# fabriceo/AVDSP

Hardware: AMD Instinct MI355X
Metric: Msamples/s (all ch) biquad+FIR chain (higher is better)
Workload: dtype f64; 1 GPU; north: 4096 ch x (16 biquads + 4096-tap FIR), block 1024 frames, DSP_FORMAT 6; 4096 ch in total, 4096 ch/GPU by dspRuntimeSetShard(rank, 1), no data-path collective; channels=4096, channels_per_gpu=4096, taps=4096, block=1024, format=6, overlap=1, ready_words=-1, ready_mode=2, side_by_side=1, streams_remade=0, cu_split=0, fir_split=0, fir_launch=-1, fir_lean=-1, ring_wait=1

## Files before the change

### avdsp_amd/csrc/avdsp_kernels.hip

```cpp
#include <hip/hip_runtime.h>
#include <hip/hip_ext.h>
#include <atomic>
#include <chrono>
#include <mutex>
#include <thread>

#include <cstdarg>
#include <cstdio>
#include <cstring>
#include <type_traits>
#include <utility>
#include <vector>
#include <algorithm>

#include "avdsp_hip.h"
#include "avdsp_format.h"

namespace {

thread_local char g_err[512];
thread_local bool g_err_ready = false;

int set_err(const char *fmt, ...)
{
// ... 1367 lines not shown

template <int FMT>
__device__ __forceinline__ void fir_append_input(const FirArgs &a, const avdsp_chain &c, int cid)
{
    const int B = a.io.nframes;
    const unsigned *inp = a.io.in + (c.in_io - a.io.in_base);
    for (int q = threadIdx.x; q < B; q += blockDim.x) {
        unsigned raw = inp[(size_t)q * a.io.in_stride];
        if constexpr (FMT == 6) raw = ftz_bits(raw);
        ring_put(a.ring, cid, q, ftz_bits(narrow_stage<FMT>(load_stage<FMT>(raw, c.load_mode, c.gain_bits))));
    }
    __syncthreads();
}

struct ChunkRegs { float h[kHRegs], x[kWRegs]; };

__device__ __forceinline__ int fir_win_slot(int u, int tid)
{
    const int idx = u * kBlock + tid, i = idx & 15, t = idx >> 4;
    return 16 * (16 * (t >> 4) + i) + (t & 15);
}

__device__ __forceinline__ void fir_chunk_fetch(const FirArgs &a, const avdsp_chain &c, int cid, int mlo, ChunkRegs &r)
{
    const int T = c.fir_taps, B = a.io.nframes, tid = threadIdx.x;
    const float *taps = reinterpret_cast<const float *>(a.buf + c.fir_coef_word);
    const float *ringrow = ring_row(a.ring, cid);
    const int rmask = a.ring.R - 1, wlen = fir_win_len(a.gpc), woff = fir_win_off(a.gpc);
#pragma unroll
    for (int u = 0; u < kHRegs; u++) { const int t = mlo + u * kBlock + tid; r.h[u] = (t >= 0 && t < T) ? taps[t] : 0.0f; }
#pragma unroll
    for (int u = 0; u < kWRegs; u++) {
        const int w = fir_win_slot(u, tid), q = w - mlo - woff;
        r.x[u] = (w < wlen && q < B) ? ringrow[(a.ring.wpos + q) & rmask] : 0.0f;
    }
}

__device__ __forceinline__ void fir_chunk_to_lds(const FirArgs &a, const ChunkRegs &r, double *hs, double *xs, int row)
{
    const int tid = threadIdx.x, hlen = fir_hs_len(a.gpc), wlen = fir_win_len(a.gpc);
#pragma unroll
    for (int u = 0; u < kHRegs; u++) { const int i = u * kBlock + tid; if (i < hlen) hs[i] = mulop(r.h[u]); }
#pragma unroll
    for (int u = 0; u < kWRegs; u++) { const int w = fir_win_slot(u, tid); if (w < wlen) xs[win_pos(w, row)] = mulop(r.x[u]); }
}

typedef double v4f64 __attribute__((ext_vector_type(4)));
typedef double v2f64 __attribute__((ext_vector_type(2)));

template <int FMT, int NG>
__global__ __launch_bounds__(kBlock, NG == 1 ? 5 : 4) void fir_mfma(const FirArgs a)
{
    extern __shared__ __attribute__((aligned(16))) double lds[];
    const int slot = xcd_remap(blockIdx.x, a.per_xcd);
    if (slot >= a.ngroup) return;
    const int cid = a.group[slot];
    const avdsp_chain c = a.chains[cid];
    double *hs = lds, *xs = lds + a.hs_cap;
    const int row = a.win_row, gpc = a.gpc;
    const int T = c.fir_taps, B = a.io.nframes;
    if (c.nsec == 0) fir_append_input<FMT>(a, c, cid);

    const int lane = threadIdx.x & 63, wave = threadIdx.x >> 6;
    const int ij = lane & 15, k = lane >> 4;
    const bool busy = wave * kTileFrames < B;
    const double *hp = hs + k + ij;
    const double *xp[4];
    const int f0 = 16 * 16 * wave + fir_win_off(gpc) - k;
#pragma unroll
    for (int s = 0; s < 4; s++) xp[s] = xs + win_pos(f0 - 4 * s, row) + ij;
    v4f64 acc = {0.0, 0.0, 0.0, 0.0};

    double ha[4 * NG], xa[4 * NG], hb[4 * NG], xb[4 * NG];
    auto load_set = [&](double *h, double *x, int g) {
#pragma unroll
        for (int q = 0; q < NG; q++)
#pragma unroll
            for (int s = 0; s < 4; s++) { h[4 * q + s] = hp[16 * (g + q) + 4 * s]; x[4 * q + s] = xp[s][-(g + q)]; }
    };
    auto mfma_set = [&](const double *h, const double *x) {
#pragma unroll
        for (int u = 0; u < 4 * NG; u++) acc = __builtin_amdgcn_mfma_f64_16x16x4f64(h[u], x[u], acc, 0, 0, 0);
    };

    const int total_groups = (T + 15 + 15) >> 4;
    const int phase = (blockIdx.x >> 8) & 3;
    int glen = max(NG, (gpc * (phase + 1) / 4) / NG * NG);
    ChunkRegs regs;
    fir_chunk_fetch(a, c, cid, -15, regs);
    for (int g0 = 0; g0 < total_groups; g0 += glen, glen = gpc) {
        __syncthreads();
        fir_chunk_to_lds(a, regs, hs, xs, row);
        __syncthreads();
        if (g0 + glen < total_groups) fir_chunk_fetch(a, c, cid, -15 + 16 * (g0 + glen), regs);
        if (busy) {
            const int ng = min(glen, total_groups - g0);
            const int nsets = (ng + NG - 1) / NG;
            load_set(ha, xa, 0);
            int st = 0;
            for (; st + 2 <= nsets; st += 2) {
                load_set(hb, xb, NG * (st + 1));
                __builtin_amdgcn_sched_barrier(0);
                mfma_set(ha, xa);
                __builtin_amdgcn_sched_barrier(0);
                load_set(ha, xa, NG * (st + 2));
                __builtin_amdgcn_sched_barrier(0);
                mfma_set(hb, xb);
                __builtin_amdgcn_sched_barrier(0);
            }
            if (st < nsets) mfma_set(ha, xa);
        }
    }
#pragma unroll
    for (int r = 0; r < 4; r++) {
        const int n = 16 * (16 * wave + ij) + k + 4 * r;
        if (n < B) {
            unsigned word = store_stage<FMT>(acc[r], c.sat, a.io.store_mask);
            if constexpr (FMT == 6) word = ftz_bits(word);
            emit_out(a.io, c, n, word);
        }
    }
}


constexpr int kTapsLead = 64;
constexpr int kTapsTail = 384;
__host__ __device__ inline int taps64_pitch(int max_taps) { return (kTapsLead + max_taps + kTapsTail + 1) & ~1; }

template <int R, bool BIG = false> struct TileGeom {
    static_assert(!BIG || R == 1, "long chunks: one row tile");
    static constexpr int NR = 16 * R;
    static constexpr int FW = 256 * R;
    static constexpr int WPC = 4 / R;
    static constexpr int QD = 4 * (R - 1);
    static constexpr int CKMAX = R == 4 ? 96 : R == 2 ? 128 : BIG ? 320 : 160;
    static constexpr int ROW = R == 4 ? 23 : R == 2 ? 33 : BIG ? 97 : 57;
    static constexpr int HNEED = 4 * CKMAX + 16 * (R - 1) + 28;
    static constexpr int HLEN = (HNEED + 127) / 128 * 128;
    static constexpr int WLEN = NR * ROW + (NR * ROW & 1);
    static constexpr int LDS_DOUBLES = 2 * HLEN + WLEN;
    static constexpr int NW = (NR * ROW + 63) / 64;
};
static_assert(TileGeom<4>::ROW >= 16 + (4 * (TileGeom<4>::CKMAX - 1) + 63) / 64 && TileGeom<2>::ROW >= 16 + (4 * (TileGeom<2>::CKMAX - 1) + 31) / 32 &&
              TileGeom<1>::ROW >= 16 + (4 * (TileGeom<1>::CKMAX - 1) + 15) / 16 &&
              TileGeom<1, true>::ROW >= 16 + (4 * (TileGeom<1, true>::CKMAX - 1) + 15) / 16, "window rows hold a chunk");

struct FirTileArgs {
    int *buf; const avdsp_chain *chains; const int *group; int ngroup; Ring ring; int per_xcd;
    const double *taps64; int pitch64;
    BlockIO io;
    unsigned *ready; unsigned seq; unsigned *timeouts;
    int ready_acquire;
    int wpc_shift;
#ifdef AVDSP_FIR_STAMPS
    unsigned long long *stamps;
#endif
};
#ifdef AVDSP_FIR_STAMPS
#define FIR_STAMP(i) do { if (lane == 0 && (i) <= 30) a.stamps[(size_t)(blockIdx.x * 4 + stamp_row) * 32 + (i)] = __builtin_amdgcn_s_memtime(); } while (0)
#define FIR_STAMP_CHUNK() do { if (stamp_i <= 21) FIR_STAMP(stamp_i); stamp_i++; } while (0)
#define FIR_REALTIME(i) do { if (lane == 0) a.stamps[(size_t)(blockIdx.x * 4 + stamp_row) * 32 + (i)] = __builtin_amdgcn_s_memrealtime(); } while (0)
#else
#define FIR_STAMP(i) do { } while (0)
#define FIR_STAMP_CHUNK() do { } while (0)
#define FIR_REALTIME(i) do { } while (0)
#endif

template <int R, bool BIG = false> __device__ __forceinline__ constexpr int win_off(int j)
{
    constexpr int NR = 16 * R;
    return ((NR - (4 * j) % NR) % NR) * TileGeom<R, BIG>::ROW - (4 * j + NR - 1) / NR + (64 / NR - 1);
}

template <int FMT, int R, bool BIG = false, bool SPLIT = false, bool LEAN = true>
__global__ __launch_bounds__(kBlock, 2) void fir_tile(const FirTileArgs a)
{
    static_assert(!SPLIT || (R == 1 && !BIG), "the tap split: one row tile, ordinary chunks");
    using G = TileGeom<R, BIG>;
    constexpr int NR = G::NR;
    extern __shared__ __attribute__((aligned(16))) double lds[];
    if constexpr (LEAN) flush_f32_subnormals_like_the_reference();
    const int lane = threadIdx.x & 63, wv = threadIdx.x >> 6;
    const int B = a.io.nframes;
    const int blk = xcd_remap(blockIdx.x, a.per_xcd);
    const int wsh = SPLIT ? (G::WPC == 4 ? 2 : G::WPC == 2 ? 1 : 0) : a.wpc_shift;
    {
        FirArgs fa{};
        fa.ring = a.ring; fa.io = a.io;
        for (int q = 0; q < (SPLIT ? 1 : 4 >> wsh); q++) {
            const int sl = SPLIT ? blk >> 1 : blk * (4 >> wsh) + q;
            if (sl < a.ngroup) {
                const int ci = a.group[sl];
                const avdsp_chain cc = a.chains[ci];
                if (cc.nsec == 0) fir_append_input<FMT>(fa, cc, ci);
            }
        }
        __syncthreads();
    }
    const int unit = SPLIT ? (blk * 4 + wv) >> 1 : blk * 4 + wv;
    [[maybe_unused]] const int half = (blk * 4 + wv) & 1;
    const int slot = unit >> wsh, F0 = (unit & ((1 << wsh) - 1)) * G::FW;
    [[maybe_unused]] int *xchg = reinterpret_cast<int *>(lds + (size_t)4 * G::LDS_DOUBLES);
    if (slot >= a.ngroup || F0 >= B) {
        if constexpr (R >= 2) {
            if (lane == 0) xchg[wv] = -1;
            __syncthreads();
        }
        if constexpr (SPLIT) __syncthreads();
        return;
    }
    [[maybe_unused]] const int stamp_row = wv;
    FIR_STAMP(0); FIR_REALTIME(29);
#ifdef AVDSP_FIR_STAMPS
    if (lane == 0) a.stamps[(size_t)(blockIdx.x * 4 + wv) * 32 + 31] = ((unsigned long long)__builtin_amdgcn_s_getreg((4 << 0) | (0 << 6) | (31 << 11)) << 32) |
                                                                       __builtin_amdgcn_s_getreg((20 << 0) | (0 << 6) | (3 << 11));
#endif
    const int cid = __builtin_amdgcn_readfirstlane(a.group[slot]);
    const avdsp_chain c = a.chains[cid];
    const int T = __builtin_amdgcn_readfirstlane(c.fir_taps);
    if (a.ready && c.nsec) chain_ready_wait(a.ready, cid, a.seq, a.timeouts, a.ready_acquire != 0);
    double *hs = lds + (size_t)wv * G::LDS_DOUBLES, *ws = hs + 2 * G::HLEN;
    const double *hbuf = a.taps64 + (size_t)cid * a.pitch64;
    const float *ringrow = ring_row(a.ring, cid);
    const int rmask = a.ring.R - 1;

    const int i16 = lane & 15, k = lane >> 4;
    const int Sall = (((T + NR + 3) >> 2) + 15) & ~15;
    const int Sb = SPLIT && half ? ((Sall >> 1) + 15) & ~15 : 0;
    const int S = SPLIT && !half ? ((Sall >> 1) + 15) & ~15 : Sall;
    const int nch = max(1, (S - Sb + G::CKMAX - 1) / G::CKMAX);
    const int ck = max(16, (((S - Sb + nch - 1) / nch) + 15) & ~15);

    v4f64 acc[R];
#pragma unroll
    for (int r = 0; r < R; r++) acc[r] = v4f64{0.0, 0.0, 0.0, 0.0};

    const int wrow = lane % NR, went = lane / NR;
    float wreg[G::NW];
    const char *ringbytes = reinterpret_cast<const char *>(ringrow);
    const unsigned rmaskb = (unsigned)rmask << 2;
    auto win_fetch = [&](int s0, int ckc) {
        const int JT = (4 * (ckc - 1) + NR - 1) / NR;
        const unsigned b0 = (unsigned)(a.ring.wpos + F0 - 3 + NR * (went + 1 - 4 * s0 / NR - JT) + wrow) << 2;
        if constexpr (LEAN) {
            const char *p0 = ringbytes + (b0 & rmaskb);
#pragma unroll
            for (int t = 0; t < G::NW; t++) wreg[t] = *reinterpret_cast<const float *>(p0 + 256 * t);
        } else {
#pragma unroll
            for (int t = 0; t < G::NW; t++) wreg[t] = *reinterpret_cast<const float *>(ringbytes + ((b0 + 256u * t) & rmaskb));
        }
    };
    auto win_store = [&](double *wdst) {
        double *wp = wdst + wrow * G::ROW + went;
        bool odd = false;
#pragma unroll
        for (int t = 0; t < G::NW; t++)
            if (t * 64 + 63 < NR * G::ROW || lane + t * 64 < NR * G::ROW) {
                if constexpr (!LEAN) odd |= __builtin_amdgcn_classf(wreg[t], 0x297);
                wp[t * (64 / NR)] = (double)wreg[t];
            }
        if constexpr (!LEAN) {
            if (__builtin_expect(__ballot(odd) != 0, 0)) {
#pragma unroll
                for (int t = 0; t < G::NW; t++)
                    if (t * 64 + 63 < NR * G::ROW || lane + t * 64 < NR * G::ROW) wp[t * (64 / NR)] = mulop(wreg[t]);
            }
        }
    };
    auto dma16 = [&](const char *sbase, unsigned voff, unsigned lds_addr) __attribute__((always_inline)) {
        unsigned keep;
        asm volatile("s_mov_b32 %[k], m0\n\t"
                     "s_mov_b32 m0, %[d]\n\t"
                     "s_nop 0\n\t"
                     "global_load_lds_dwordx4 %[v], %[s]\n\t"
                     "s_mov_b32 m0, %[k]"
                     : [k] "=&s"(keep) : [v] "v"(voff), [s] "s"(sbase), [d] "s"(lds_addr) : "memory");
    };
    const unsigned hs_addr = __builtin_amdgcn_readfirstlane((unsigned)(size_t)(__attribute__((address_space(3))) char *)hs);
    const unsigned lane16 = (unsigned)lane * 16u;
    auto taps_dma = [&](int which, int s0, int ckc) {
        const unsigned long long sv = reinterpret_cast<unsigned long long>(hbuf + (kTapsLead - 16) - 16 * (R - 1) + 4 * s0);
        const char *src = reinterpret_cast<const char *>(((unsigned long long)(unsigned)__builtin_amdgcn_readfirstlane((unsigned)(sv >> 32)) << 32) |
                                                         (unsigned long long)(unsigned)__builtin_amdgcn_readfirstlane((unsigned)sv));
        const int np = (4 * ckc + 16 * (R - 1) + 28) / 2;
        const unsigned dst = hs_addr + (unsigned)which * (unsigned)(G::HLEN * 8);
#pragma unroll
        for (int t = 0; t < G::HLEN / 128; t++)
            if (64 * t < np) {
                if constexpr (LEAN) dma16(src + 1024 * t, lane16, dst + 1024u * t);
                else {
                    const int pi = lane + 64 * t;
                    __builtin_amdgcn_global_load_lds(src + 16 * (pi < np ? pi : np - 1), (__attribute__((address_space(3))) char *)(hs + which * G::HLEN) + 1024 * t, 16, 0, 0);
                }
            }
    };

    double q[16], bq[4];
    auto chunk_begin = [&](const double *hp, const double *wp) {
#pragma unroll
        for (int j = 0; j < G::QD; j++) q[(16 - G::QD + j) & 15] = hp[4 * j];
        q[0] = hp[16 * (R - 1)]; q[1] = hp[16 * (R - 1) + 4];
        bq[0] = wp[win_off<R, BIG>(0)]; bq[1] = wp[win_off<R, BIG>(1)];
    };
    auto kstep = [&](const double *hg, const double *wg, auto jc) {
        constexpr int j = decltype(jc)::value;
        q[(j + 2) & 15] = hg[4 * (j + 2)];
        bq[(j + 2) & 3] = j + 2 < 16 ? wg[win_off<R, BIG>((j + 2) & 15)] : (wg - 64 / NR)[win_off<R, BIG>((j + 2) & 15)];
        __builtin_amdgcn_sched_barrier(0);
#pragma unroll
        for (int r = 0; r < R; r++)
            acc[r] = __builtin_amdgcn_mfma_f64_16x16x4f64(q[(j - 4 * (R - 1 - r)) & 15], bq[j & 3], acc[r], 0, 0, 0);
        __builtin_amdgcn_sched_barrier(0);
    };
    auto group16 = [&](const double *hg, const double *wg) {
        kstep(hg, wg, std::integral_constant<int, 0>{});  kstep(hg, wg, std::integral_constant<int, 1>{});
        kstep(hg, wg, std::integral_constant<int, 2>{});  kstep(hg, wg, std::integral_constant<int, 3>{});
        kstep(hg, wg, std::integral_constant<int, 4>{});  kstep(hg, wg, std::integral_constant<int, 5>{});
        kstep(hg, wg, std::integral_constant<int, 6>{});  kstep(hg, wg, std::integral_constant<int, 7>{});
        kstep(hg, wg, std::integral_constant<int, 8>{});  kstep(hg, wg, std::integral_constant<int, 9>{});
        kstep(hg, wg, std::integral_constant<int, 10>{}); kstep(hg, wg, std::integral_constant<int, 11>{});
        kstep(hg, wg, std::integral_constant<int, 12>{}); kstep(hg, wg, std::integral_constant<int, 13>{});
        kstep(hg, wg, std::integral_constant<int, 14>{}); kstep(hg, wg, std::integral_constant<int, 15>{});
    };

    win_fetch(Sb, min(ck, S - Sb));
    taps_dma(0, Sb, min(ck, S - Sb));
    [[maybe_unused]] int stamp_i = 1;
    int cur = 0;
    for (int s0 = Sb; s0 < S; s0 += ck, cur ^= 1) {
        const int ckc = min(ck, S - s0);
        const int JT = (4 * (ckc - 1) + NR - 1) / NR;
        __builtin_amdgcn_wave_barrier();
        FIR_STAMP_CHUNK();
        win_store(ws);
        if (s0 == Sb + ck) FIR_STAMP(24);
        asm volatile("s_waitcnt vmcnt(0)" ::: "memory");
        __builtin_amdgcn_fence(__ATOMIC_RELEASE, "wavefront");
        __builtin_amdgcn_wave_barrier();
        if (s0 == Sb + ck) FIR_STAMP(25);
        if (s0 + ckc < S) {
            win_fetch(s0 + ckc, min(ck, S - s0 - ckc));
            if (s0 == Sb + ck) FIR_STAMP(26);
            taps_dma(cur ^ 1, s0 + ckc, min(ck, S - s0 - ckc));
        }
        if (s0 == Sb + ck) FIR_STAMP(27);
        const double *hp = hs + cur * G::HLEN + k + i16;
        const double *wp = ws + (3 - k) * G::ROW + i16 + JT - (64 / NR - 1);
        chunk_begin(hp, wp);
        FIR_STAMP_CHUNK();
        for (int g = 0; g < ckc / 16; g++) group16(hp + 16 * (R - 1) + 64 * g, wp - g * (64 / NR));
        FIR_STAMP_CHUNK();
    }
    FIR_STAMP(23);
    if constexpr (LEAN) {
        bool odd = false;
#pragma unroll
        for (int r = 0; r < R; r++)
#pragma unroll
            for (int v = 0; v < 4; v++)
                odd |= F0 + NR * i16 + 16 * r + 4 * v + k < B && ((unsigned long long)__double_as_longlong(acc[r][v]) >> 52 & 0x7FF) == 0x7FF;
        if (__builtin_expect(__ballot(odd) != 0, 0)) {
            const float *ftaps = reinterpret_cast<const float *>(a.buf + c.fir_coef_word);
            const int Sfrom = SPLIT ? (half ? 4 * Sb - NR : 0) : 0, Sto = SPLIT && !half ? min(T, 4 * S - NR) : T;
#pragma unroll
            for (int r = 0; r < R; r++)
#pragma unroll
                for (int v = 0; v < 4; v++) {
                    const int n = F0 + NR * i16 + 16 * r + 4 * v + k;
                    double sum = 0.0;
                    for (int tp = max(Sfrom, 0); tp < Sto; tp++)
                        sum = __builtin_fma(mulop(ringrow[(a.ring.wpos + n - tp) & rmask]), mulop(ftaps[tp]), sum);
                    acc[r][v] = sum;
                }
        }
    }
    if constexpr (R >= 2) {
        constexpr int CH = R, WPC = G::WPC;
        const bool four = R == 2 && wsh == 0;
        unsigned *mine = reinterpret_cast<unsigned *>(hs);
        unsigned w16[4 * R];
#pragma unroll
        for (int r = 0; r < R; r++)
#pragma unroll
            for (int v = 0; v < 4; v++) {
                unsigned word = store_stage<FMT>(acc[r][v], c.sat, a.io.store_mask);
                if constexpr (FMT == 6) word = ftz_bits(word);
                w16[4 * r + v] = word;
                mine[(NR + 1) * i16 + 16 * r + 4 * v + k] = word;
            }
        if (lane == 0) xchg[wv] = c.n_out == 1 ? c.out_io[0] : -1;
        __syncthreads();
        const int o0 = xchg[0];
        const int chn = four ? 4 : CH;
        bool together = o0 >= 0 && ((o0 - a.io.out_base) & (chn - 1)) == 0 && (a.io.out_stride & (chn - 1)) == 0 &&
                        (reinterpret_cast<size_t>(a.io.out) & (4 * chn - 1)) == 0;
#pragma unroll
        for (int w = 1; w < 4; w++) together = together && xchg[w] == o0 + (w >> wsh);
        if (together && four) {
            if constexpr (R == 2) {
                const unsigned *reg = reinterpret_cast<const unsigned *>(lds);
#pragma unroll
                for (int qf = 0; qf < 2; qf++) {
                    const int f = (int)threadIdx.x + 256 * qf;
                    if (f < B) {
                        const int at = (NR + 1) * (f / NR) + f % NR;
                        unsigned o[4];
#pragma unroll
                        for (int j = 0; j < 4; j++) o[j] = reg[(size_t)j * (2 * G::LDS_DOUBLES) + at];
                        unsigned *dst = a.io.out + (size_t)f * a.io.out_stride + (o0 - a.io.out_base);
                        *reinterpret_cast<uint4 *>(dst) = make_uint4(o[0], o[1], o[2], o[3]);
                    }
                }
            }
        } else if (together) {
            const unsigned *reg = reinterpret_cast<const unsigned *>(lds);
#pragma unroll
            for (int qf = 0; qf < 4; qf++) {
                const int f = (int)threadIdx.x + 256 * qf;
                if (f < B) {
                    const int ti = f / G::FW, fl = f - ti * G::FW;
                    const int at = (NR + 1) * (fl / NR) + fl % NR;
                    unsigned o[CH];
#pragma unroll
                    for (int j = 0; j < CH; j++) o[j] = reg[(size_t)(j * WPC + ti) * (2 * G::LDS_DOUBLES) + at];
                    unsigned *dst = a.io.out + (size_t)f * a.io.out_stride + (o0 - a.io.out_base);
                    if constexpr (CH == 4) *reinterpret_cast<uint4 *>(dst) = make_uint4(o[0], o[1], o[2], o[3]);
                    else *reinterpret_cast<uint2 *>(dst) = make_uint2(o[0], o[1]);
                }
            }
        } else {
#pragma unroll
            for (int r = 0; r < R; r++)
#pragma unroll
                for (int v = 0; v < 4; v++) {
                    const int n = F0 + NR * i16 + 16 * r + 4 * v + k;
                    if (n < B) emit_out(a.io, c, n, w16[4 * r + v]);
                }
        }
    } else {
        if constexpr (SPLIT) {
            v4f64 *park = reinterpret_cast<v4f64 *>(lds + (size_t)(wv | 1) * G::LDS_DOUBLES);
            if (half) park[lane] = acc[0];
            __syncthreads();
            if (half) return;
            acc[0] += park[lane];
        }
#pragma unroll
        for (int r = 0; r < R; r++)
#pragma unroll
            for (int v = 0; v < 4; v++) {
                const int n = F0 + NR * i16 + 16 * r + 4 * v + k;
                if (n < B) {
                    unsigned word = store_stage<FMT>(acc[r][v], c.sat, a.io.store_mask);
                    if constexpr (FMT == 6) word = ftz_bits(word);
                    emit_out(a.io, c, n, word);
                }
            }
    }
    FIR_STAMP(30); FIR_REALTIME(28);
}


template <int R> struct SharedGeom {
    static constexpr int CK = 64;
    static constexpr int FW = 64 * R;
    static constexpr int NU = 4 * CK + 48 * R;
    static constexpr int CP = (NU - 2 + 31) / 32 * 32 + 2;
    static constexpr int HNEED = 4 * CK + 16 * R;
    static constexpr int HLEN = (HNEED + 127) / 128 * 128;
    static constexpr int NWR = (NU + 63) / 64;
    static constexpr int LDS_DOUBLES = 2 * HLEN + 16 * CP;
};
static_assert(SharedGeom<1>::LDS_DOUBLES * 8 <= 64 * 1024 && SharedGeom<2>::LDS_DOUBLES * 8 <= 64 * 1024 &&
              SharedGeom<4>::LDS_DOUBLES * 8 <= 64 * 1024, "two fir_shared workgroups per CU");
static_assert(SharedGeom<4>::HLEN / 128 <= 4, "one taps piece per wave");

struct SharedTile { int group, first, n, taps; };
struct FirSharedArgs {
    int *buf; const avdsp_chain *chains; const int *ids; const SharedTile *tiles; int ntiles; int nfb; Ring ring; int per_xcd;
    const double *taps64; int pitch64;
    BlockIO io;
};

template <int FMT, int R>
__global__ __launch_bounds__(kBlock, 2) void fir_shared(const FirSharedArgs a)
{
    using G = SharedGeom<R>;
    extern __shared__ __attribute__((aligned(16))) double lds[];
    flush_f32_subnormals_like_the_reference();
    const int L = xcd_remap(blockIdx.x, a.per_xcd);
    if (L >= a.ntiles * a.nfb) return;
    const int lane = threadIdx.x & 63, wv = threadIdx.x >> 6;
    const int B = a.io.nframes;
    const SharedTile tile = a.tiles[L / a.nfb];
    const int F0 = (L % a.nfb) * G::FW, F0w = F0 + 16 * R * wv;
    const int T = tile.taps;
    double *hs = lds, *ws = lds + 2 * G::HLEN;
    const double *hbuf = a.taps64 + (size_t)tile.group * a.pitch64;
    const int rmask = a.ring.R - 1;

    const char *srow[4];
#pragma unroll
    for (int q = 0; q < 4; q++) {
// ... 1556 lines not shown
    return (size_t)(*hs_cap + 16 * *row) * sizeof(double);
}

Ring plan_ring(const Plan &pl) { return Ring{pl.d_ring, pl.ring_R, pl.wpos, pl.d_ring64}; }

hipEvent_t take_event(avdsp_hip_prog *prog)
{
    if (!prog->free_events.empty()) { hipEvent_t e = prog->free_events.back(); prog->free_events.pop_back(); return e; }
    hipEvent_t e = nullptr;
    if (hipEventCreateWithFlags(&e, hipEventDisableSystemFence) != hipSuccess) return nullptr;
    return e;
}

struct ProfileScope {
    avdsp_hip_prog *prog; hipStream_t stream; int kind; bool on = false; hipEvent_t a = nullptr;
    ProfileScope(avdsp_hip_prog *p, hipStream_t s, int k) : prog(p), stream(s), kind(k)
    {
        on = (prog->profile >> kind & 1u) && prog->profile_seen[kind & 7]++ % (unsigned)prog->profile_stride == 0;
    }
    void keep(hipEvent_t s, hipEvent_t e, bool pair)
    {
        if (prog->spans.size() >= 65536) {
            for (size_t i = 0; i < 32768; i++) {
                for (int k = 0; k < avdsp_hip_prog::kAhead; k++)
                    if (prog->ev_fir_now[k] == prog->spans[i].b) { (void)hipEventSynchronize(prog->spans[i].b); prog->ev_fir_now[k] = prog->ev_fir[k]; prog->ev_fir_set[k] = false; }
                prog->free_events.push_back(prog->spans[i].a); prog->free_events.push_back(prog->spans[i].b);
            }
            prog->spans.erase(prog->spans.begin(), prog->spans.begin() + 32768);
        }
        prog->spans.push_back({kind, s, e, pair});
    }
    bool ride(hipEvent_t &s, hipEvent_t &e)
    {
        if (!on) return false;
        s = take_event(prog); e = take_event(prog);
        if (!s || !e) { if (s) prog->free_events.push_back(s); if (e) prog->free_events.push_back(e); return false; }
        keep(s, e, false);
        prog->last_ride_stop = e;
        return true;
    }
    void begin() { if (on && !a && (a = take_event(prog))) (void)hipEventRecord(a, stream); }
    ~ProfileScope()
    {
        if (!a) return;
        hipEvent_t b = take_event(prog);
        if (!b) { prog->free_events.push_back(a); return; }
        (void)hipEventRecord(b, stream);
        keep(a, b, true);
    }
};

template <typename Args>
int launch_timed(ProfileScope &scope, const void *fn, dim3 grid, dim3 block, size_t lds, hipStream_t stream, Args &a, hipEvent_t stop = nullptr)
{
    void *kargs[] = {(void *)&a};
    hipEvent_t s = nullptr, e = nullptr;
    if (stop) { scope.begin(); HIP_TRY(hipExtLaunchKernel(fn, grid, block, kargs, lds, stream, nullptr, stop, 0)); return 0; }
    if (scope.ride(s, e)) { HIP_TRY(hipExtLaunchKernel(fn, grid, block, kargs, lds, stream, s, e, 0)); return 0; }
    if (scope.kind == AVDSP_KERNEL_FIR && scope.prog->fir_mode_now == 2) {
        avdsp_hip_prog *pg = scope.prog;
        const unsigned k = (pg->launch_ev_next++ & 7u) * 2;
        for (unsigned j = k; j < k + 2; j++) if (!pg->launch_ev[j]) HIP_TRY(hipEventCreate(&pg->launch_ev[j]));
        HIP_TRY(hipExtLaunchKernel(fn, grid, block, kargs, lds, stream, pg->launch_ev[k], pg->launch_ev[k + 1], 0));
        return 0;
    }
    HIP_TRY(hipLaunchKernel(fn, grid, block, kargs, lds, stream));
    return 0;
}

#ifdef AVDSP_BQ_STAMPS
static unsigned long long *g_bq_stamps = nullptr; static int g_bq_stamp_waves = 0;
extern "C" int avdsp_hip_debug_bq_stamps(unsigned long long *host_out, int max_waves)
{
    if (!g_bq_stamps) return 0;
    const int n = g_bq_stamp_waves < max_waves ? g_bq_stamp_waves : max_waves;
    if (hipDeviceSynchronize() != hipSuccess) return -1;
    if (hipMemcpy(host_out, g_bq_stamps, (size_t)n * 32 * 8, hipMemcpyDeviceToHost) != hipSuccess) return -1;
    return n;
}
#endif

template <int FMT>
int launch_biquad(avdsp_hip_prog *prog, Plan &pl, const Plan::Group &g, const int *ids, int n, BlockIO io,
                  int biquad_impl, hipStream_t stream, hipEvent_t stop = nullptr, bool with_ready = false)
{
    ProfileScope scope(prog, stream, AVDSP_KERNEL_BIQUAD);
    BiquadArgs a{};
    a.buf = prog->d_buf; a.chains = pl.d_chains; a.sec_coef = pl.d_sec_coef; a.sec_state = pl.d_sec_state;
    a.group = ids; a.ngroup = n; a.nsec = g.nsec; a.ring = plan_ring(pl); a.io = io;
    a.ready = with_ready ? pl.d_ready : nullptr; a.seq = pl.seq;
#ifdef AVDSP_BQ_STAMPS
    {
        static unsigned long long *d_stamps = nullptr;
        if (!d_stamps) { HIP_TRY(hipMalloc((void **)&d_stamps, (size_t)65536 * 4 * 32 * 8)); }
        HIP_TRY(hipMemsetAsync(d_stamps, 0, (size_t)65536 * 4 * 32 * 8, stream));
        a.stamps = d_stamps; g_bq_stamps = d_stamps; g_bq_stamp_waves = ((n * g.P + kBlock - 1) / kBlock + 7) / 8 * 8 * 4;
    }
#endif
    if (biquad_impl == 0 || g.P > 64) {
        scope.begin();
        hipLaunchKernelGGL(biquad_simple<FMT>, dim3((n + 63) / 64), dim3(64), 0, stream, a);
        if (stop) HIP_TRY(hipEventRecord(stop, stream));
    } else if (biquad_impl == 1 && g.P == 16 && g.d_rows) {
        if constexpr (FMT == 2) {
            const int nblk = (n + 15) / 16;
            a.rows = g.d_rows; a.lanes = g.d_lanes;
            a.per_xcd = (nblk + 7) / 8;
            if (launch_timed(scope, (const void *)biquad_row_i64, dim3(a.per_xcd * 8), dim3(kBlock), 0, stream, a, stop)) return -1;
        } else {
            const int nblk = (n + 15) / 16;
            a.rows = g.d_rows; a.lanes = g.d_lanes;
            a.per_xcd = (nblk + 7) / 8;
            const void *fn = (const void *)biquad_row<FMT>;
            if constexpr (FMT == 4) { if (!(g.all_fir || g.raw_out)) fn = (const void *)biquad_row<4, true>; }
            if (launch_timed(scope, fn, dim3(a.per_xcd * 8), dim3(kBlock), 0, stream, a, stop)) return -1;
        }
    } else {
        const int cpb = kBlock / g.P;
        const int nblk = (n + cpb - 1) / cpb;
        a.per_xcd = (nblk + 7) / 8;
        const void *fn = g.P == 1 ? (const void *)biquad_pipe<FMT, 1> : g.P == 2 ? (const void *)biquad_pipe<FMT, 2> : g.P == 4 ? (const void *)biquad_pipe<FMT, 4>
                       : g.P == 8 ? (const void *)biquad_pipe<FMT, 8> : g.P == 16 ? (const void *)biquad_pipe<FMT, 16> : g.P == 32 ? (const void *)biquad_pipe<FMT, 32>
                       : (const void *)biquad_pipe<FMT, 64>;
        if (launch_timed(scope, fn, dim3(a.per_xcd * 8), dim3(kBlock), 0, stream, a, stop)) return -1;
    }
    HIP_TRY(hipGetLastError());
    return 0;
}

#ifdef AVDSP_FIR_STAMPS
static unsigned long long *g_fir_stamps = nullptr; static int g_fir_stamp_waves = 0;
extern "C" int avdsp_hip_debug_fir_stamps(unsigned long long *host_out, int max_waves)
{
    if (!g_fir_stamps) return 0;
    const int n = std::min(max_waves, g_fir_stamp_waves);
    if (hipDeviceSynchronize() != hipSuccess) return -1;
    if (hipMemcpy(host_out, g_fir_stamps, (size_t)n * 32 * 8, hipMemcpyDeviceToHost) != hipSuccess) return -1;
    return n;
}
#endif

template <int FMT, int R, bool BIG = false, bool SPLIT = false>
int launch_fir_tile(avdsp_hip_prog *prog, Plan &pl, const int *ids, int n, BlockIO io, hipStream_t stream, ProfileScope &scope, bool wait_ready, hipEvent_t stop = nullptr, bool lean = true)
{
    FirTileArgs a{};
    a.buf = prog->d_buf; a.chains = pl.d_chains; a.group = ids; a.ngroup = n;
    a.ring = plan_ring(pl); a.io = io; a.taps64 = pl.d_taps64; a.pitch64 = pl.pitch64;
    if (wait_ready) { a.ready = pl.d_ready; a.seq = pl.seq; a.timeouts = prog->d_ready_timeouts; a.ready_acquire = prog->ready_mode_now != 2 || prog->overlap >= 2; }
    constexpr int kWpc = TileGeom<R, BIG>::WPC;
    const int tiles = (io.nframes + TileGeom<R, BIG>::FW - 1) / TileGeom<R, BIG>::FW;
    const bool quarters = SPLIT || (BIG && n <= (prog->num_cus > 0 ? prog->num_cus : 256));
    const int wpc = quarters ? kWpc : tiles <= 1 ? 1 : tiles <= 2 ? std::min(2, kWpc) : kWpc;
    a.wpc_shift = wpc == 4 ? 2 : wpc == 2 ? 1 : 0;
    const int nwg = (n * wpc * (SPLIT ? 2 : 1) + 3) / 4;
    a.per_xcd = (nwg + 7) / 8;
    const size_t lds = (size_t)4 * TileGeom<R, BIG>::LDS_DOUBLES * sizeof(double) + 64;
#ifdef AVDSP_FIR_STAMPS
    static unsigned long long *d_stamps = nullptr;
    if (!d_stamps) { HIP_TRY(hipMalloc((void **)&d_stamps, (size_t)8192 * 4 * 32 * 8)); }
    HIP_TRY(hipMemsetAsync(d_stamps, 0, (size_t)8192 * 4 * 32 * 8, stream));
    a.stamps = d_stamps;
    g_fir_stamps = d_stamps; g_fir_stamp_waves = a.per_xcd * 8 * 4;
#endif
    return launch_timed(scope, lean ? (const void *)fir_tile<FMT, R, BIG, SPLIT, true> : (const void *)fir_tile<FMT, R, BIG, SPLIT, false>,
                        dim3(a.per_xcd * 8), dim3(kBlock), lds, stream, a, stop);
}


template <int FMT, int R>
int launch_fir_stream(avdsp_hip_prog *prog, Plan &pl, const int *ids, int n, BlockIO io, hipStream_t stream)
{
    if (!pl.d_ring64) {
        HIP_TRY(hipDeviceSynchronize());
        HIP_TRY(hipMalloc((void **)&pl.d_ring64, (size_t)pl.nchains * 2 * pl.ring_R * sizeof(double)));
        RingConvArgs ca{prog->d_buf, pl.d_chains, pl.d_fir_ids, pl.n_fir, plan_ring(pl)};
        hipLaunchKernelGGL(ring_widen, dim3(pl.n_fir), dim3(kBlock), 0, stream, ca);
        HIP_TRY(hipGetLastError());
    }
    FirTileArgs a{};
    a.buf = prog->d_buf; a.chains = pl.d_chains; a.group = ids; a.ngroup = n;
    a.ring = plan_ring(pl); a.io = io; a.taps64 = pl.d_taps64; a.pitch64 = pl.pitch64;
    if (pl.n_fir_only) {
        const long long total = (long long)n * io.nframes;
        hipLaunchKernelGGL(fir_feed<FMT>, dim3((unsigned)std::min<long long>((total + kBlock - 1) / kBlock, 4096)), dim3(kBlock), 0, stream, a);
        HIP_TRY(hipGetLastError());
    }
    const int tiles = (io.nframes + StreamGeom<R>::FW - 1) / StreamGeom<R>::FW;
    const int nwg = std::min((n * tiles + 3) / 4, prog->num_cus > 0 ? prog->num_cus : 256);
    a.per_xcd = (nwg + 7) / 8;
    const size_t lds = (size_t)4 * StreamGeom<R>::LDS_DOUBLES * sizeof(double) + 64;
#ifdef AVDSP_FIR_STAMPS
    static unsigned long long *d_stamps = nullptr;
    if (!d_stamps) { HIP_TRY(hipMalloc((void **)&d_stamps, (size_t)8192 * 4 * 32 * 8)); }
    HIP_TRY(hipMemsetAsync(d_stamps, 0, (size_t)8192 * 4 * 32 * 8, stream));
    a.stamps = d_stamps;
    g_fir_stamps = d_stamps; g_fir_stamp_waves = a.per_xcd * 8 * 4;
#endif
    hipLaunchKernelGGL((fir_stream<FMT, R>), dim3(a.per_xcd * 8), dim3(kStreamBlock), lds, stream, a);
    HIP_TRY(hipGetLastError());
    return 0;
}

template <int FMT, int R, bool BIG = false>
int launch_fir_flow(avdsp_hip_prog *prog, Plan &pl, const int *ids, int n, BlockIO io, hipStream_t stream, ProfileScope &scope, bool wait_ready, hipEvent_t stop)
{
    if (!pl.d_ring64) {
        HIP_TRY(hipDeviceSynchronize());
        HIP_TRY(hipMalloc((void **)&pl.d_ring64, (size_t)pl.nchains * 2 * pl.ring_R * sizeof(double)));
        RingConvArgs ca{prog->d_buf, pl.d_chains, pl.d_fir_ids, pl.n_fir, plan_ring(pl)};
        hipLaunchKernelGGL(ring_widen, dim3(pl.n_fir), dim3(kBlock), 0, stream, ca);
        HIP_TRY(hipGetLastError());
    }
    FirTileArgs a{};
    a.buf = prog->d_buf; a.chains = pl.d_chains; a.group = ids; a.ngroup = n;
    a.ring = plan_ring(pl); a.io = io; a.taps64 = pl.d_taps64; a.pitch64 = pl.pitch64;
    if (wait_ready) { a.ready = pl.d_ready; a.seq = pl.seq; a.timeouts = prog->d_ready_timeouts; a.ready_acquire = prog->ready_mode_now != 2 || prog->overlap >= 2; }
    a.wpc_shift = FlowGeom<R, BIG>::WPC == 4 ? 2 : FlowGeom<R, BIG>::WPC == 2 ? 1 : 0;
    const int nwg = (n * FlowGeom<R, BIG>::WPC + 3) / 4;
    a.per_xcd = (nwg + 7) / 8;
    const size_t lds = (size_t)4 * FlowGeom<R, BIG>::LDS_DOUBLES * sizeof(double) + 64;
#ifdef AVDSP_FIR_STAMPS
    static unsigned long long *d_stamps = nullptr;
    if (!d_stamps) { HIP_TRY(hipMalloc((void **)&d_stamps, (size_t)8192 * 4 * 32 * 8)); }
    HIP_TRY(hipMemsetAsync(d_stamps, 0, (size_t)8192 * 4 * 32 * 8, stream));
    a.stamps = d_stamps;
    g_fir_stamps = d_stamps; g_fir_stamp_waves = a.per_xcd * 8 * 4;
#endif
    return launch_timed(scope, (const void *)fir_flow<FMT, R, BIG>, dim3(a.per_xcd * 8), dim3(kBlock), lds, stream, a, stop);
}

int ensure_private_taps(avdsp_hip_prog *prog, Plan &pl, hipStream_t stream)
{
    if (pl.d_taps64 || !pl.n_fir) return 0;
    HIP_TRY(hipMalloc((void **)&pl.d_taps64, (size_t)pl.nchains * pl.pitch64 * sizeof(double)));
    Taps64Args ta{prog->d_buf, pl.d_chains, pl.d_fir_ids, pl.d_taps64, pl.pitch64, 0};
    hipLaunchKernelGGL(taps_to_f64, dim3(pl.n_fir), dim3(kBlock), 0, stream, ta);
    HIP_TRY(hipGetLastError());
    return 0;
}

bool shared_path(const avdsp_hip_prog *prog, const Plan &pl, int fir_impl)
{
    return pl.n_sh_groups > 0 && prog->fir_shared && fir_impl == 1 && !prog->overlap && !prog->fir_split && pl.instances <= 1;
}

template <int FMT, int R>
int launch_fir_shared_r(avdsp_hip_prog *prog, Plan &pl, BlockIO io, hipStream_t stream, ProfileScope &scope)
{
    FirSharedArgs a{};
    a.buf = prog->d_buf; a.chains = pl.d_chains; a.ids = pl.d_sh_ids; a.tiles = pl.d_sh_tiles; a.ntiles = pl.n_sh_tiles;
    a.nfb = (io.nframes + SharedGeom<R>::FW - 1) / SharedGeom<R>::FW;
    a.ring = plan_ring(pl); a.taps64 = pl.d_sh_taps64; a.pitch64 = pl.pitch64; a.io = io;
    const long long nwg = (long long)a.ntiles * a.nfb;
    a.per_xcd = (int)((nwg + 7) / 8);
    return launch_timed(scope, (const void *)fir_shared<FMT, R>, dim3(a.per_xcd * 8), dim3(kBlock), (size_t)SharedGeom<R>::LDS_DOUBLES * sizeof(double), stream, a);
}

template <int FMT>
int launch_fir_shared(avdsp_hip_prog *prog, Plan &pl, BlockIO io, hipStream_t stream)
{
    if constexpr (FMT != 4 && FMT != 6) { (void)prog; (void)pl; (void)io; (void)stream; return set_err("fir_shared: formats 4 and 6 only"); }
    else {
        if (pl.n_sh_feed) {
            FirTileArgs f{};
            f.buf = prog->d_buf; f.chains = pl.d_chains; f.group = pl.d_sh_feed; f.ngroup = pl.n_sh_feed; f.ring = plan_ring(pl); f.io = io;
            const long long total = (long long)pl.n_sh_feed * io.nframes;
            hipLaunchKernelGGL(fir_feed<FMT>, dim3((unsigned)std::min<long long>((total + kBlock - 1) / kBlock, 4096)), dim3(kBlock), 0, stream, f);
            HIP_TRY(hipGetLastError());
        }
        ProfileScope scope(prog, stream, AVDSP_KERNEL_FIR);
        int rows = prog->fir_rows;
        if (rows != 1 && rows != 2 && rows != 4) {
            double best = 1e30;
            rows = 1;
            for (int r : {4, 2, 1}) {
                if (r > 1 && 32 * r >= io.nframes) continue;
                const long long waves = (long long)pl.n_sh_tiles * 4 * ((io.nframes + 64 * r - 1) / (64 * r));
                const double cost = (double)((waves + 2047) / 2048) * r / (r == 4 ? 0.90 : r == 2 ? 0.84 : 0.79);
                if (cost < best - 1e-9) { best = cost; rows = r; }
            }
        }
        while (rows > 1 && 32 * rows >= io.nframes) rows >>= 1;
        if constexpr (FMT == 4) {
            return rows >= 2 ? launch_fir_shared_r<FMT, 2>(prog, pl, io, stream, scope) : launch_fir_shared_r<FMT, 1>(prog, pl, io, stream, scope);
        } else {
            return rows == 4 ? launch_fir_shared_r<FMT, 4>(prog, pl, io, stream, scope)
                 : rows == 2 ? launch_fir_shared_r<FMT, 2>(prog, pl, io, stream, scope)
                             : launch_fir_shared_r<FMT, 1>(prog, pl, io, stream, scope);
        }
    }
}

template <int FMT>
int launch_fir(avdsp_hip_prog *prog, Plan &pl, const int *ids, int n, BlockIO io, int fir_impl, hipStream_t stream, bool wait_ready = false, hipEvent_t stop = nullptr)
{
    if constexpr (FMT == 2) { (void)prog; (void)pl; (void)ids; (void)n; (void)io; (void)fir_impl; (void)stream; (void)wait_ready; (void)stop; return 0; }
    else {
        if (ensure_private_taps(prog, pl, stream)) return -1;
        ProfileScope scope(prog, stream, AVDSP_KERNEL_FIR);
        if (fir_impl == 4) {
            int rows = prog->fir_rows;
            if (rows != 1 && rows != 2 && rows != 4) rows = n >= 2048 ? 4 : n >= 1024 ? 2 : 1;
            while (rows > 1 && 128 * rows >= io.nframes) rows >>= 1;
            if (rows == 1 && (long long)n * ((io.nframes + 255) / 256) <= 1024 && prog->fir_rows != 1)
                return launch_fir_flow<FMT, 1, true>(prog, pl, ids, n, io, stream, scope, wait_ready, stop);
            return rows == 4 ? launch_fir_flow<FMT, 4>(prog, pl, ids, n, io, stream, scope, wait_ready, stop)
// ... 2131 lines not shown
```

Baseline: 8334 Msamples/s.

## Skip zero-tap MFMA steps at FIR edges and overlap tap DMA with ready wait

The FIR tile kernel now predicates MFMA steps by tap index. Steps in the first group whose taps precede the filter start, and steps past the last real tap, are skipped instead of multiplying zero-padded coefficients. The tap DMA for the first chunk is issued before the biquad-ready spin-wait so the copy overlaps the wait. The input-append prologue is skipped when no chain is FIR-only. This adds edge-case template variants and a waitcnt in chunk_begin, so code size and scheduling change in exchange for fewer wasted MFMAs and less startup latency.

```diff
diff --git a/avdsp_amd/csrc/avdsp_kernels.hip b/avdsp_amd/csrc/avdsp_kernels.hip
--- a/avdsp_amd/csrc/avdsp_kernels.hip
+++ b/avdsp_amd/csrc/avdsp_kernels.hip
@@ -1543,6 +1543,7 @@
     unsigned *ready; unsigned seq; unsigned *timeouts;
     int ready_acquire;
     int wpc_shift;
+    int all_cascaded;
 #ifdef AVDSP_FIR_STAMPS
     unsigned long long *stamps;
 #endif
@@ -1575,7 +1576,7 @@
     const int B = a.io.nframes;
     const int blk = xcd_remap(blockIdx.x, a.per_xcd);
     const int wsh = SPLIT ? (G::WPC == 4 ? 2 : G::WPC == 2 ? 1 : 0) : a.wpc_shift;
-    {
+    if (!a.all_cascaded) {
         FirArgs fa{};
         fa.ring = a.ring; fa.io = a.io;
         for (int q = 0; q < (SPLIT ? 1 : 4 >> wsh); q++) {
@@ -1609,7 +1610,6 @@
     const int cid = __builtin_amdgcn_readfirstlane(a.group[slot]);
     const avdsp_chain c = a.chains[cid];
     const int T = __builtin_amdgcn_readfirstlane(c.fir_taps);
-    if (a.ready && c.nsec) chain_ready_wait(a.ready, cid, a.seq, a.timeouts, a.ready_acquire != 0);
     double *hs = lds + (size_t)wv * G::LDS_DOUBLES, *ws = hs + 2 * G::HLEN;
     const double *hbuf = a.taps64 + (size_t)cid * a.pitch64;
     const float *ringrow = ring_row(a.ring, cid);
@@ -1693,30 +1693,41 @@
         for (int j = 0; j < G::QD; j++) q[(16 - G::QD + j) & 15] = hp[4 * j];
         q[0] = hp[16 * (R - 1)]; q[1] = hp[16 * (R - 1) + 4];
         bq[0] = wp[win_off<R, BIG>(0)]; bq[1] = wp[win_off<R, BIG>(1)];
+        if constexpr (LEAN) {
+            __builtin_amdgcn_s_waitcnt(0xC07F);
+            __builtin_amdgcn_sched_barrier(0);
+        }
     };
-    auto kstep = [&](const double *hg, const double *wg, auto jc) {
-        constexpr int j = decltype(jc)::value;
+    const int slast = (T - 1 + NR) >> 2;
+    auto kstep = [&](const double *hg, const double *wg, auto jc, auto ec, [[maybe_unused]] int sg) {
+        constexpr int j = decltype(jc)::value, EDGE = decltype(ec)::value;
+        if (EDGE == 2 && sg + j > slast) return false;
         q[(j + 2) & 15] = hg[4 * (j + 2)];
         bq[(j + 2) & 3] = j + 2 < 16 ? wg[win_off<R, BIG>((j + 2) & 15)] : (wg - 64 / NR)[win_off<R, BIG>((j + 2) & 15)];
         __builtin_amdgcn_sched_barrier(0);
 #pragma unroll
-        for (int r = 0; r < R; r++)
-            acc[r] = __builtin_amdgcn_mfma_f64_16x16x4f64(q[(j - 4 * (R - 1 - r)) & 15], bq[j & 3], acc[r], 0, 0, 0);
+        for (int r = 0; r < R; r++) {
+            const int first = 4 * (R - 1 - r);
+            if (EDGE == 0 || (EDGE == 1 && j >= first) || (EDGE == 2 && (unsigned)(sg + j - first) <= (unsigned)(slast - 4 * r - first)))
+                acc[r] = __builtin_amdgcn_mfma_f64_16x16x4f64(q[(j - 4 * (R - 1 - r)) & 15], bq[j & 3], acc[r], 0, 0, 0);
+        }
         __builtin_amdgcn_sched_barrier(0);
+        return true;
     };
-    auto group16 = [&](const double *hg, const double *wg) {
-        kstep(hg, wg, std::integral_constant<int, 0>{});  kstep(hg, wg, std::integral_constant<int, 1>{});
-        kstep(hg, wg, std::integral_constant<int, 2>{});  kstep(hg, wg, std::integral_constant<int, 3>{});
-        kstep(hg, wg, std::integral_constant<int, 4>{});  kstep(hg, wg, std::integral_constant<int, 5>{});
-        kstep(hg, wg, std::integral_constant<int, 6>{});  kstep(hg, wg, std::integral_constant<int, 7>{});
-        kstep(hg, wg, std::integral_constant<int, 8>{});  kstep(hg, wg, std::integral_constant<int, 9>{});
-        kstep(hg, wg, std::integral_constant<int, 10>{}); kstep(hg, wg, std::integral_constant<int, 11>{});
-        kstep(hg, wg, std::integral_constant<int, 12>{}); kstep(hg, wg, std::integral_constant<int, 13>{});
-        kstep(hg, wg, std::integral_constant<int, 14>{}); kstep(hg, wg, std::integral_constant<int, 15>{});
+    auto group16 = [&](const double *hg, const double *wg, auto ec, int sg) {
+        (void)(kstep(hg, wg, std::integral_constant<int, 0>{}, ec, sg) && kstep(hg, wg, std::integral_constant<int, 1>{}, ec, sg) &&
+               kstep(hg, wg, std::integral_constant<int, 2>{}, ec, sg) && kstep(hg, wg, std::integral_constant<int, 3>{}, ec, sg) &&
+               kstep(hg, wg, std::integral_constant<int, 4>{}, ec, sg) && kstep(hg, wg, std::integral_constant<int, 5>{}, ec, sg) &&
+               kstep(hg, wg, std::integral_constant<int, 6>{}, ec, sg) && kstep(hg, wg, std::integral_constant<int, 7>{}, ec, sg) &&
+               kstep(hg, wg, std::integral_constant<int, 8>{}, ec, sg) && kstep(hg, wg, std::integral_constant<int, 9>{}, ec, sg) &&
+               kstep(hg, wg, std::integral_constant<int, 10>{}, ec, sg) && kstep(hg, wg, std::integral_constant<int, 11>{}, ec, sg) &&
+               kstep(hg, wg, std::integral_constant<int, 12>{}, ec, sg) && kstep(hg, wg, std::integral_constant<int, 13>{}, ec, sg) &&
+               kstep(hg, wg, std::integral_constant<int, 14>{}, ec, sg) && kstep(hg, wg, std::integral_constant<int, 15>{}, ec, sg));
     };
 
+    taps_dma(0, Sb, min(ck, S - Sb));
+    if (a.ready && c.nsec) chain_ready_wait(a.ready, cid, a.seq, a.timeouts, a.ready_acquire != 0);
     win_fetch(Sb, min(ck, S - Sb));
-    taps_dma(0, Sb, min(ck, S - Sb));
     [[maybe_unused]] int stamp_i = 1;
     int cur = 0;
     for (int s0 = Sb; s0 < S; s0 += ck, cur ^= 1) {
@@ -1740,7 +1751,11 @@
         const double *wp = ws + (3 - k) * G::ROW + i16 + JT - (64 / NR - 1);
         chunk_begin(hp, wp);
         FIR_STAMP_CHUNK();
-        for (int g = 0; g < ckc / 16; g++) group16(hp + 16 * (R - 1) + 64 * g, wp - g * (64 / NR));
+        const int gfull = min(ckc / 16, ((slast - 4 * (R - 1) - 15 - s0) >> 4) + 1);
+        int g = 0;
+        if (R > 1 && s0 == 0 && gfull > 0) { group16(hp + 16 * (R - 1), wp, std::integral_constant<int, 1>{}, 0); g = 1; }
+        for (; g < gfull; g++) group16(hp + 16 * (R - 1) + 64 * g, wp - g * (64 / NR), std::integral_constant<int, 0>{}, 0);
+        for (; g < ckc / 16; g++) group16(hp + 16 * (R - 1) + 64 * g, wp - g * (64 / NR), std::integral_constant<int, 2>{}, s0 + 16 * g);
         FIR_STAMP_CHUNK();
     }
     FIR_STAMP(23);
@@ -3603,6 +3618,7 @@
     const bool quarters = SPLIT || (BIG && n <= (prog->num_cus > 0 ? prog->num_cus : 256));
     const int wpc = quarters ? kWpc : tiles <= 1 ? 1 : tiles <= 2 ? std::min(2, kWpc) : kWpc;
     a.wpc_shift = wpc == 4 ? 2 : wpc == 2 ? 1 : 0;
+    a.all_cascaded = pl.n_fir_only == 0;
     const int nwg = (n * wpc * (SPLIT ? 2 : 1) + 3) / 4;
     a.per_xcd = (nwg + 7) / 8;
     const size_t lds = (size_t)4 * TileGeom<R, BIG>::LDS_DOUBLES * sizeof(double) + 64;
```

New measurement: 8480 Msamples/s (median of 6 runs). 1.02x the previous value.
